# zhuker/lamejs

Hardware: NVIDIA H100
Metric: encoded audio seconds/sec (44.1kHz stereo 128kbps CBR) (higher is better)
Workload: dtype f64

## Files before the change

lamejs_b200/csrc/k_quant.cuh:

```cuda
#ifndef MP3B200_K_QUANT_CUH
#define MP3B200_K_QUANT_CUH
#include <stddef.h>
#include "mp3_device.cuh"
#include "mp3_tables.h"
#include "k_psy.cuh"

#define Q_LARGE_BITS 100000
#define Q_IXMAX 8206
#define Q_FULL 0xffffffffu

struct GranuleInfoDev {
  int global_gain, part2_3_length, part2_length, big_values, count1, scalefac_compress;
  int table_select[3], region0_count, region1_count, preflag, scalefac_scale, count1table_select, block_type;
  int subblock_gain[4];
  int count1bits, sfbmax, sfbdivide, sfb_lmax, psymax, psy_lmax, sfb_smin, max_nonzero_coeff;
  int scalefac[MP3_SFBMAX];
  int slen[4];
  int part_row;
  int pad_;
  double xrpow_max;
};
struct QuantFrameState {
  int stream, rel_frame;
  int in_old[2], in_step[2];
  int out_old[2], out_step[2];
  int bs_gain0[2], bs_step0[2];
  int used0[2];
  unsigned long long bs_hash[2][2];
  int scfsi[2][4];
  int redo;
  int valid;
};
#define Q_R0(ch) (1 << (ch))
#define Q_R1S(ch) (4 << (ch))
#define Q_R1(ch) (16 << (ch))
#define Q_R0_ANY 3
#define Q_R1_ANY 48
#define Q_R1S_ANY 12
struct GcPrep { float xmin[MP3_SFBMAX]; int have, mnz, block_type; double xrpow_max; };

__device__ unsigned short g_huff_code[1666];
__device__ unsigned char g_huff_len[1666];
__constant__ int c_huff_off[34];
__constant__ int c_huff_xlen[34];
__device__ int g_t32l[16];
__device__ int g_t33l[16];
__constant__ int c_slen1_n[16];
__constant__ int c_slen2_n[16];
__device__ int g_slen_n[2][16];
__device__ int g_scale_tab[2][16];
__device__ unsigned int g_cat_tab[8][256];
__constant__ int c_slen1_tab[16];
__constant__ int c_slen2_tab[16];
__constant__ int c_huf_noesc[15];

static int quant_upload_constants() {
  static const int t32l[16] = {1, 5, 5, 7, 5, 8, 7, 9, 5, 7, 7, 9, 7, 9, 9, 10};
  static const int t33l[16] = {4, 5, 5, 6, 5, 6, 6, 7, 5, 6, 6, 7, 6, 7, 7, 8};
  static const int s1n[16] = {1, 1, 1, 1, 8, 2, 2, 2, 4, 4, 4, 8, 8, 8, 16, 16};
  static const int s2n[16] = {1, 2, 4, 8, 1, 2, 4, 8, 2, 4, 8, 2, 4, 8, 4, 8};
  static const int s1t[16] = {0, 0, 0, 0, 3, 1, 1, 1, 2, 2, 2, 3, 3, 3, 4, 4};
  static const int s2t[16] = {0, 1, 2, 3, 0, 1, 2, 3, 1, 2, 3, 1, 2, 3, 2, 3};
  static const int ss[16] = {0, 18, 36, 54, 54, 36, 54, 72, 54, 72, 90, 72, 90, 108, 108, 126};
  static const int sl[16] = {0, 10, 20, 30, 33, 21, 31, 41, 32, 42, 52, 43, 53, 63, 64, 74};
  static const int hn[15] = {1, 2, 5, 7, 7, 10, 10, 13, 13, 13, 13, 13, 13, 13, 13};
#define UP(sym, src) if (cudaMemcpyToSymbol(sym, src, sizeof(src)) != cudaSuccess) return -100
  UP(g_huff_code, MP3_HUFF_CODE); UP(g_huff_len, MP3_HUFF_LEN); UP(c_huff_off, MP3_HUFF_OFF);
  UP(c_huff_xlen, MP3_HUFF_XLEN);
  UP(g_t32l, t32l); UP(g_t33l, t33l); UP(c_slen1_n, s1n); UP(c_slen2_n, s2n);
  UP(c_slen1_tab, s1t); UP(c_slen2_tab, s2t); UP(c_huf_noesc, hn);
  {
    static int sn[2][16], st[2][16];
    static unsigned int ct[8][256];
    for (int k = 0; k < 16; k++) { sn[0][k] = s1n[k]; sn[1][k] = s2n[k]; st[0][k] = sl[k]; st[1][k] = ss[k]; }
    static const int fam[6] = {1, 2, 5, 7, 10, 13};
    for (int x = 0; x < 16; x++) for (int y = 0; y < 16; y++) {
      const int q = x * 16 + y;
      for (int c = 0; c < 6; c++) {
        const int t1 = fam[c], xl = MP3_HUFF_XLEN[t1];
        unsigned a = 0, b = 0, d = 0;
        if (x < xl && y < xl) {
          const int i = x * xl + y;
          if (c == 0) a = b = d = MP3_HUFF_LEN[MP3_HUFF_OFF[1] + i];
          else if (c == 1) { a = MP3_HUFF_TABLE23[i] >> 16; b = d = MP3_HUFF_TABLE23[i] & 0xffff; }
          else if (c == 2) { a = MP3_HUFF_TABLE56[i] >> 16; b = d = MP3_HUFF_TABLE56[i] & 0xffff; }
          else { a = MP3_HUFF_LEN[MP3_HUFF_OFF[t1] + i]; b = MP3_HUFF_LEN[MP3_HUFF_OFF[t1 + 1] + i]; d = MP3_HUFF_LEN[MP3_HUFF_OFF[t1 + 2] + i]; }
        }
        ct[c][q] = a | (b << 11) | (d << 22);
      }
      { const unsigned a = MP3_HUFF_LARGETBL[q] >> 16, b = MP3_HUFF_LARGETBL[q] & 0xffff; ct[6][q] = a | (b << 11) | (b << 22); }
      ct[7][q] = 0;
    }
    UP(g_slen_n, sn); UP(g_scale_tab, st); UP(g_cat_tab, ct);
  }
#undef UP
  return 0;
}

struct __align__(16) GcWork {
  float xrpow[576];
  short ixw[576];
  short* ixg;
  GranuleInfoDev w, b;
  const Mp3Geo* geo;
  float xmin[MP3_SFBMAX], distort[MP3_SFBMAX];
  int pn_step[MP3_SFBMAX]; float pn_noise[MP3_SFBMAX], pn_noise_log[MP3_SFBMAX];
  int pn_global_gain, pn_sfb_count1;
  unsigned char mode[MP3_SFBMAX + 1];
  short nstart[MP3_SFBMAX], nlen[MP3_SFBMAX];
  int scratch[8];
  double dscratch[4];
  __align__(16) float xr[576];
};
struct __align__(16) WarpShared {
  double ath[6];
  int scfsi[4];
  GcWork wk;
};
#define Q_STRIDE_NOXR ((int)((offsetof(WarpShared, wk) + offsetof(GcWork, xr) + 15) & ~(size_t)15))
static_assert((offsetof(WarpShared, wk) + offsetof(GcWork, xr)) % 16 == 0 && (offsetof(WarpShared, wk) + offsetof(GcWork, xrpow)) % 16 == 0 &&
              (offsetof(WarpShared, wk) + offsetof(GcWork, ixw)) % 16 == 0 && sizeof(WarpShared) % 16 == 0, "rows are moved as 16-byte vectors");
#ifndef Q_SLIM_BLOCKS
#define Q_SLIM_BLOCKS 9
#endif

#define LANE (threadIdx.x & 31)
#ifdef Q_TASKSTAT
__device__ int g_taskstat[1 << 16][8];
#endif
#ifdef Q_STATS
__device__ unsigned long long g_qstats[16];
#define QSTAT(i) do { if (LANE == 0) atomicAdd(&g_qstats[i], 1ull); } while (0)
#else
#define QSTAT(i) do { } while (0)
#endif
#define Q_PRAGMA(x) _Pragma(#x)
#define Q_UNROLL(n) Q_PRAGMA(unroll n)
#ifndef Q_RT_UNROLL
#define Q_RT_UNROLL 1
#endif
#ifndef Q_CB_UNROLL
#define Q_CB_UNROLL 1
#endif
#ifndef Q_CN_UNROLL
#define Q_CN_UNROLL 2
#endif
#ifndef Q_HELPER
#define Q_HELPER __forceinline__
#endif
#ifndef Q_SPEC_START
#define Q_SPEC_START 180
#endif
#ifndef Q_SPEC_STEP
#define Q_SPEC_STEP 32
#endif
#ifndef Q_SPEC_GR1_STEP
#define Q_SPEC_GR1_STEP 2
#endif
#ifndef Q_SPEC_FOLD
#define Q_SPEC_FOLD 1
#endif
#ifndef Q_MIN_BLOCKS
#define Q_MIN_BLOCKS 14
#endif
__device__ __noinline__ double q_log10(double x) { return m3_log10(x); }
__device__ __noinline__ double q_pow(double x, double y) { return m3_pow(x, y); }
__device__ __forceinline__ int wmax(int v) { return __reduce_max_sync(Q_FULL, v); }
__device__ __forceinline__ int wsum(int v) { return __reduce_add_sync(Q_FULL, v); }
__device__ __forceinline__ unsigned wsumu(unsigned v) { return __reduce_add_sync(Q_FULL, v); }

struct RegionClass { int cat; unsigned lin; int t1, t2; };
__device__ Q_HELPER RegionClass region_class(int mx) {
  RegionClass rc;
  rc.lin = 0; rc.t2 = 0;
  if (mx == 0) { rc.cat = 7; rc.t1 = 0; }
  else if (mx <= 15) {
    rc.t1 = c_huf_noesc[mx - 1];
    rc.cat = mx <= 3 ? mx - 1 : (mx <= 5 ? 3 : (mx <= 7 ? 4 : 5));
  } else {
    const int n = 32 - __clz(mx - 15);
    rc.t2 = 24 + (int)((0x7777665432100000ull >> (4 * n)) & 15ull);
    rc.t1 = max(rc.t2 - 8, 16 + (int)((0x7777766554432100ull >> (4 * n)) & 15ull));
    const unsigned la = (unsigned)c_huff_xlen[rc.t1], lb = (unsigned)c_huff_xlen[rc.t2];
    rc.lin = la | (lb << 11) | (lb << 22);
    rc.cat = 6;
// ... 149 lines not shown
    for (int p = lane; p < 288; p += 32) {
      unsigned v = 0;
      if (2 * p < qend) {
        const float2 xp = *reinterpret_cast<const float2*>(&wk->xrpow[2 * p]);
        double x0 = (double)xp.x * istep, x1 = (double)xp.y * istep;
        x0 += (double)__ldg(&T->adj43[js_trunc<DOM_TRUNC_QUANT>(x0)]);
        x1 += (double)__ldg(&T->adj43[js_trunc<DOM_TRUNC_QUANT>(x1)]);
        v = (unsigned)js_trunc<DOM_TRUNC_QUANT>(x0) | ((unsigned)js_trunc<DOM_TRUNC_QUANT>(x1) << 16);
        DOMAIN_MISS(DOM_PACK_SEARCH, x0 >= 32768.0 || x1 >= 32768.0);
        if (v != 0 && p < i0h) top = 2 * p + 2;
      }
      iw32[p] = v;
    }
    __syncwarp();
    return noquant_count_bits_w(T, ix, gi, wk, false, top);
  }
  const bool prev_data_use = use_prev && (gi->global_gain == wk->pn_global_gain);
  const bool calc_step = prev_data_use || gi->block_type == BT_NORM;
  int term = sfbmax + 1;
#pragma unroll 1
  for (int s0 = 0; s0 <= sfbmax; s0 += 32) {
    const int sfb = s0 + lane;
    int md = 0, trunc_here = 0;
    if (sfb <= sfbmax) {
      const int jst = wk->geo->start[sfb];
      const int step = calc_step ? sfb_step(gi, wk, sfb) : -1;
      if (prev_data_use && wk->pn_step[sfb] == step) md = 0;
      else {
        if (jst + wk->geo->width[sfb] > mnz) trunc_here = 1;
        md = (use_prev && wk->pn_sfb_count1 > 0 && sfb >= wk->pn_sfb_count1 && wk->pn_step[sfb] > 0 && step >= wk->pn_step[sfb]) ? 2 : 1;
      }
      wk->mode[sfb] = (unsigned char)md;
      wk->nstart[sfb] = jst;
    }
    const unsigned m = __ballot_sync(Q_FULL, trunc_here);
    if (m && term == sfbmax + 1) term = s0 + __ffs(m) - 1;
  }
  __syncwarp();
  int zero_from = 576;
  if (term <= sfbmax) {
    const int term_len = mnz - wk->nstart[term] + 1;
    zero_from = term_len > 0 ? ((term_len & 1) ? mnz : mnz + 1) : mnz;
    if (lane == 0) wk->mode[term] = 1;
  }
  __syncwarp();
  const double compare01 = T->cmp01_over_istep[gi->global_gain];
  int top = 0;
Q_UNROLL(Q_CB_UNROLL)
  for (int p = lane; p < 288; p += 32) {
    const int i = 2 * p;
    unsigned v;
    if (i >= zero_from) { v = 0; iw32[p] = 0; }
    else {
      const int md = wk->mode[wk->geo->sfb_of_line[i]];
      const bool z1 = (i + 1) >= zero_from;
      if (md == 0) {
        v = iw32[p];
        if (z1) { v &= 0xffffu; iw32[p] = v; }
      } else {
        const float2 xp = *reinterpret_cast<const float2*>(&wk->xrpow[i]);
        unsigned v0, v1;
        if (md == 2) { v0 = (compare01 > (double)xp.x) ? 0u : 1u; v1 = (compare01 > (double)xp.y) ? 0u : 1u; }
        else {
          double x0 = (double)xp.x * istep, x1 = (double)xp.y * istep;
          x0 += (double)__ldg(&T->adj43[js_trunc<DOM_TRUNC_QUANT>(x0)]);
          x1 += (double)__ldg(&T->adj43[js_trunc<DOM_TRUNC_QUANT>(x1)]);
          v0 = (unsigned)js_trunc<DOM_TRUNC_QUANT>(x0); v1 = (unsigned)js_trunc<DOM_TRUNC_QUANT>(x1);
          DOMAIN_MISS(DOM_PACK_OUTER, x0 >= 32768.0 || x1 >= 32768.0);
        }
        if (z1) v1 = 0;
        v = v0 | (v1 << 16);
        iw32[p] = v;
      }
    }
    if (v != 0 && p < i0h) top = 2 * p + 2;
  }
  __syncwarp();
  return noquant_count_bits_w(T, ix, gi, wk, use_prev, top);
}

struct NoiseRes { int over_count; double over_SSD, max_noise; int bits; };
__device__ __forceinline__ void calc_noise_w(const Mp3Tables* T, GcWork* wk, const GranuleInfoDev* gi, const short* ix, NoiseRes* res) {
  const int lane = LANE;
  const int psymax = gi->psymax, mnz = gi->max_nonzero_coeff;
  int first_trunc = psymax;
#pragma unroll 1
  for (int s0 = 0; s0 < psymax; s0 += 32) {
    const int sfb = s0 + lane;
    int crosses = 0;
    if (sfb < psymax) {
      const int j = wk->geo->start[sfb], w = wk->geo->width[sfb];
      if (wk->pn_step[sfb] == sfb_step(gi, wk, sfb)) wk->nlen[sfb] = -1;
      else { wk->nstart[sfb] = (short)j; wk->nlen[sfb] = (short)(w >> 1); crosses = (j + w) > mnz; }
    }
    const unsigned m = __ballot_sync(Q_FULL, crosses);
    if (m && first_trunc == psymax) first_trunc = s0 + __ffs(m) - 1;
  }
  __syncwarp();
  if (lane == 0 && first_trunc < psymax) {
    int j = wk->geo->start[first_trunc];
#pragma unroll 1
    for (int sfb = first_trunc; sfb < psymax; sfb++) {
      const int w = wk->geo->width[sfb];
      if (wk->nlen[sfb] < 0) { j += w; continue; }
      int l = w >> 1;
      if ((j + w) > mnz) { const int us = mnz - j + 1; l = us > 0 ? us >> 1 : 0; }
      wk->nstart[sfb] = (short)j; wk->nlen[sfb] = (short)l;
      j += 2 * l;
    }
  }
  __syncwarp();
  int over = 0, ssd = 0; double mxn = -20.0;
#pragma unroll 1
  for (int s0 = 0; s0 < psymax; s0 += 32) {
    const int sfb = s0 + lane;
    if (sfb < psymax) {
      const int s = sfb_step(gi, wk, sfb);
      const bool cached = wk->nlen[sfb] < 0;
      double noise;
      if (cached) noise = (double)wk->pn_noise[sfb];
      else {
        const double step = (double)T->pow20[s + MP3_QMAX2];
        int j = wk->nstart[sfb];
        noise = 0;
Q_UNROLL(Q_CN_UNROLL)
        for (int l = wk->nlen[sfb]; l > 0; l--, j += 2) {
          const float2 x = *reinterpret_cast<const float2*>(&wk->xr[j]);
          const unsigned q0 = reinterpret_cast<const unsigned short*>(ix)[j], q1 = reinterpret_cast<const unsigned short*>(ix)[j + 1];
          double temp;
          temp = fabs((double)x.x) - (double)__ldg(&T->pow43[q0]) * step; noise += temp * temp;
          temp = fabs((double)x.y) - (double)__ldg(&T->pow43[q1]) * step; noise += temp * temp;
        }
        wk->pn_step[sfb] = s;
        { f32s t; t = noise; wk->pn_noise[sfb] = t.v; }
      }
      noise = noise / (double)wk->xmin[sfb];
      { f32s t; t = noise; wk->distort[sfb] = t.v; }
      if (cached) noise = (double)wk->pn_noise_log[sfb];
      else {
        noise = q_log10(js_dmax(noise, 1E-20));
        { f32s t; t = noise; wk->pn_noise_log[sfb] = t.v; }
      }
      if (noise > 0.0) {
        int tmp = js_trunc<DOM_TRUNC_NOISE>(noise * 10 + .5);
        if (tmp < 1) tmp = 1;
        ssd += tmp * tmp;
        over++;
      }
      mxn = js_dmax(mxn, noise);
    }
  }
#pragma unroll 1
  for (int o = 16; o > 0; o >>= 1) {
    const double other = __shfl_xor_sync(Q_FULL, mxn, o);
    mxn = js_dmax(mxn, other);
  }
  over = wsum(over);
  if (lane == 0) wk->pn_global_gain = gi->global_gain;
  __syncwarp();
  res->over_count = over; res->over_SSD = (double)wsum(ssd); res->max_noise = mxn;
}

__device__ __forceinline__ bool scale_bitcount_w(GranuleInfoDev* gi) {
  const int lane = LANE;
  int* scalefac = gi->scalefac;
  const bool is_short = gi->block_type == BT_SHORT;
  const int sfbmax = gi->sfbmax, sfbdivide = gi->sfbdivide;
  __syncwarp();
  if (!is_short && 0 == gi->preflag) {
    const bool in = lane >= 11 && lane < 21;
    const int pt = pretab_of(lane);
    const bool ok = !in || scalefac[lane] >= pt;
    if (__all_sync(Q_FULL, ok)) {
      __syncwarp();
      if (in) scalefac[lane] -= pt;
      if (lane == 0) gi->preflag = 1;
      __syncwarp();
    }
  }
  int m1 = 0, m2 = 0;
#pragma unroll 1
  for (int sfb = lane; sfb < sfbmax; sfb += 32) {
    const int v = scalefac[sfb];
    if (sfb < sfbdivide) m1 = max(m1, v); else m2 = max(m2, v);
  }
  m1 = wmax(m1); m2 = wmax(m2);
  int key = Q_LARGE_BITS * 16 + 15;
  if (lane < 16 && m1 < __ldg(&g_slen_n[0][lane]) && m2 < __ldg(&g_slen_n[1][lane])) key = __ldg(&g_scale_tab[is_short ? 1 : 0][lane]) * 16 + lane;
  key = __reduce_min_sync(Q_FULL, key);
  const int p2 = key >> 4;
  if (lane == 0) { gi->part2_length = p2; if (p2 != Q_LARGE_BITS) gi->scalefac_compress = key & 15; }
  __syncwarp();
  return p2 == Q_LARGE_BITS;
}

__device__ __forceinline__ bool scale_bitcount_lsf_w(GranuleInfoDev* gi) {
  const int lane = LANE;
  const bool is_short = gi->block_type == BT_SHORT;
  __syncwarp();
  int m0 = 0, m1 = 0, m2 = 0, m3 = 0;
  const int n = is_short ? 36 : 21;
#pragma unroll 1
  for (int i = lane; i < n; i += 32) {
    const int v = gi->scalefac[i];
    const int p = is_short ? i / 9 : (i < 6 ? 0 : (i - 6) / 5 + 1);
    if (p == 0) m0 = max(m0, v); else if (p == 1) m1 = max(m1, v); else if (p == 2) m2 = max(m2, v); else m3 = max(m3, v);
  }
  m0 = wmax(m0); m1 = wmax(m1); m2 = wmax(m2); m3 = wmax(m3);
  const bool over = m0 > 15 || m1 > 15 || m2 > 7 || m3 > 7;
  if (!over && lane == 0) {
// ... 916 lines not shown
      if (ixq[i + 2] != 0) { p += 2; huffbits *= 2; if (QNEG(i + 2)) huffbits++; }
      if (ixq[i + 3] != 0) { p++; huffbits *= 2; if (QNEG(i + 3)) huffbits++; }
      const int len = __ldg(&g_huff_len[c_huff_off[tb] + p]);
      if (pass == 0) mybits += len;
      else { put_bits(buf, at, (unsigned)huffbits + __ldg(&g_huff_code[c_huff_off[tb] + p]), len); at += len; }
    }
  }
  __syncwarp();
}

__device__ __forceinline__ void put_header_bits(unsigned int* buf, int pos, int val, int n) {
  while (n > 0) {
    const int k = min(n, 8 - (pos & 7));
    n -= k;
    const unsigned byte = ((unsigned)(val >> n) << (8 - (pos & 7) - k)) & 0xffu;
    const int b = pos >> 3;
    atomicOr(&buf[b >> 2], byte << (24 - 8 * (b & 3)));
    pos += k;
  }
}

__device__ __noinline__ void pack_sideinfo(const Mp3Tables* T, unsigned int* buf, const GranuleInfoDev* __restrict__ fin,
                                           const int* scfsi, int padding) {
  int p = 0;
#define WH(v, n) do { put_header_bits(buf, p, (int)(v), (n)); p += (n); } while (0)
  const int nch = T->nch;
  WH(T->mpeg25 ? 0xffe : 0xfff, 12); WH(T->version, 1); WH(4 - 3, 2); WH(1, 1);
  WH(T->bitrate_index, 4); WH(T->samplerate_index, 2); WH(padding, 1); WH(0, 1);
  WH(T->mono ? 3 : 0, 2); WH(0, 2); WH(0, 1); WH(1, 1); WH(0, 2);
  if (T->version == 1) {
    WH(0, 9);
    WH(0, nch == 2 ? 3 : 5);
#pragma unroll 1
    for (int ch = 0; ch < nch; ch++) for (int b = 0; b < 4; b++) WH(scfsi[ch * 4 + b], 1);
  } else {
    WH(0, 8);
    WH(0, nch);
  }
#pragma unroll 1
  for (int gr = 0; gr < T->mode_gr; gr++) for (int ch = 0; ch < nch; ch++) {
    const GranuleInfoDev* gi = &fin[gr * nch + ch];
    WH(gi->part2_3_length + gi->part2_length, 12);
    WH(gi->big_values / 2, 9);
    WH(gi->global_gain, 8);
    WH(gi->scalefac_compress, T->version == 1 ? 4 : 9);
    int ts0 = gi->table_select[0], ts1 = gi->table_select[1], ts2 = gi->table_select[2];
    if (ts0 == 14) ts0 = 16;
    if (ts1 == 14) ts1 = 16;
    if (gi->block_type != BT_NORM) {
      WH(1, 1); WH(gi->block_type, 2); WH(0, 1);
      WH(ts0, 5); WH(ts1, 5);
      WH(gi->subblock_gain[0], 3); WH(gi->subblock_gain[1], 3); WH(gi->subblock_gain[2], 3);
    } else {
      WH(0, 1);
      if (ts2 == 14) ts2 = 16;
      WH(ts0, 5); WH(ts1, 5); WH(ts2, 5);
      WH(gi->region0_count, 4); WH(gi->region1_count, 3);
    }
    if (T->version == 1) WH(gi->preflag, 1);
    WH(gi->scalefac_scale, 1); WH(gi->count1table_select, 1);
  }
#undef WH
}

__device__ __forceinline__ int granule_budget(int nch, int mean_bits, int gr, int used0, int used1, int ch) {
  int tbits = mean_bits;
  if (gr == 1) {
    const int resv = -(used0 + (nch == 2 ? used1 : 0)) + mean_bits;
    if (resv * 10 > 0) tbits += resv;
  }
  double t = (double)tbits / nch;
  if (t > 4095) t = 4095;
  int targ = (int)t;
  const int bits = targ * nch;
  if (bits > 7680) { targ = targ * 7680; targ = (int)((double)targ / bits); }
  (void)ch;
  return targ;
}

#ifndef Q_WARPS
#define Q_WARPS 4
#endif
#ifndef Q_BLOCKS_PER_SM
#define Q_BLOCKS_PER_SM 7
#endif
#define Q_THREADS (32 * Q_WARPS)

__device__ __forceinline__ int next_task(int* counter) {
  int t = 0;
  if (LANE == 0) t = atomicAdd(counter, 1);
  return __shfl_sync(Q_FULL, t, 0);
}
template <int STRIDE = (int)sizeof(WarpShared)>
__device__ __forceinline__ WarpShared* warp_shared() {
  extern __shared__ __align__(16) unsigned char smem_raw[];
  return reinterpret_cast<WarpShared*>(smem_raw + (threadIdx.x >> 5) * STRIDE);
}
__device__ __forceinline__ void gi_init_w(GranuleInfoDev* gi, const GcPrep* __restrict__ pr) {
  __syncwarp();
  int* w = reinterpret_cast<int*>(gi);
#pragma unroll 1
  for (int i = LANE; i < (int)(sizeof(GranuleInfoDev) / 4); i += 32) w[i] = 0;
  __syncwarp();
  if (LANE == 0) {
    const int bt = pr->block_type;
    const bool is_short = bt == BT_SHORT;
    gi->global_gain = 210; gi->block_type = bt;
    gi->sfb_lmax = is_short ? 0 : 21; gi->sfb_smin = is_short ? 0 : 12; gi->psy_lmax = is_short ? 0 : 21;
    gi->psymax = is_short ? 36 : 21; gi->sfbmax = is_short ? 36 : 21; gi->sfbdivide = is_short ? 18 : 11;
    gi->max_nonzero_coeff = pr->mnz; gi->xrpow_max = pr->xrpow_max;
  }
  __syncwarp();
}
__device__ __forceinline__ void copy_row16_w(void* dst, const void* src, int nbytes) {
  __syncwarp();
  const int n = nbytes >> 4;
  int4 v[5];
#pragma unroll
  for (int k = 0; k < 5; k++) { const int i = LANE + 32 * k; if (i < n) v[k] = reinterpret_cast<const int4*>(src)[i]; }
#pragma unroll
  for (int k = 0; k < 5; k++) { const int i = LANE + 32 * k; if (i < n) reinterpret_cast<int4*>(dst)[i] = v[k]; }
  __syncwarp();
}
struct FrameGeom { int z, f, padding, frame_bytes, mean_bits; long long kabs; };
__device__ __forceinline__ FrameGeom frame_geom(const Mp3Tables* T, const StreamDesc* streams, const QuantFrameState* q) {
  FrameGeom g;
  g.z = q->stream; g.f = q->rel_frame;
  g.kabs = (long long)streams[g.z].frame0 + g.f;
  g.padding = (int)(pad_count(g.kabs, T->frac_SpF, T->samplerate) - pad_count(g.kabs - 1, T->frac_SpF, T->samplerate));
  g.frame_bytes = T->frame_bytes_nopad + g.padding;
  g.mean_bits = (8 * g.frame_bytes - T->sideinfo_len * 8) / T->mode_gr;
  return g;
}

__global__ void __launch_bounds__(Q_THREADS, Q_BLOCKS_PER_SM)
k_q_prepare(const Mp3Tables* __restrict__ T, const StreamDesc* __restrict__ streams, const float* __restrict__ xr,
            const PsyRatioDev* __restrict__ ratio, const signed char* __restrict__ bt_final, const double* __restrict__ ath_q,
            const QuantFrameState* __restrict__ qs, float* __restrict__ xrq, float* __restrict__ xrpow_g, unsigned* __restrict__ neg_g,
            GcPrep* __restrict__ prep,
            int nframes, int* __restrict__ counter) {
  WarpShared* ws = warp_shared();
  GcWork* wk = &ws->wk;
  const int lane = LANE, nch = T->nch;
  const int G = T->mode_gr;
  const int ntasks = nframes * G * nch;
#pragma unroll 1
  for (int t = next_task(counter); t < ntasks; t = next_task(counter)) {
    const int frow = t / (G * nch), rem = t - frow * G * nch, gr = rem / nch, ch = rem - gr * nch;
    const QuantFrameState* q = qs + frow;
    const int z = q->stream, f = q->rel_frame;
    const StreamDesc& sd = streams[z];
    const double ath_adjust = ath_q[frow];
    const size_t urow = (size_t)sd.unit_base + G * f + gr, gidx = urow * nch + ch;
    const int bt = bt_final[urow * 2 + ch];
    const PsyRatioDev* rt = ratio + ((size_t)sd.unit_base + z + G * f + gr) * nch + ch;
    __syncwarp();
    if (lane < 6) ws->ath[lane] = ath_adjust_dev(ath_adjust, (double)(bt == BT_SHORT ? T->ath_psfb12[lane] : T->ath_psfb21[lane]), T->ath_floor);
    __syncwarp();
    const bool have = gc_prepare_w(T, wk, ws->ath, xr + gidx * 576, bt, rt, ath_adjust);
    copy_row16_w(xrq + gidx * 576, wk->xr, 2304);
    {
      unsigned mine = 0;
#pragma unroll 1
      for (int k = 0; k < 18; k++) { const unsigned m = __ballot_sync(Q_FULL, wk->xr[lane + 32 * k] < 0.0f); if (lane == k) mine = m; }
      if (lane < 18) neg_g[gidx * 18 + lane] = mine;
    }
    copy_row16_w(xrpow_g + gidx * 576, wk->xrpow, 2304);
    GcPrep* pr = prep + gidx;
#pragma unroll 1
    for (int i = lane; i < MP3_SFBMAX; i += 32) pr->xmin[i] = wk->xmin[i];
    if (lane == 0) { pr->have = have ? 1 : 0; pr->mnz = wk->b.max_nonzero_coeff; pr->block_type = bt; pr->xrpow_max = wk->b.xrpow_max; }
  }
}

__global__ void __launch_bounds__(Q_THREADS, Q_SLIM_BLOCKS)
k_q_search(const Mp3Tables* __restrict__ T, const StreamDesc* __restrict__ streams, QuantFrameState* __restrict__ qs,
           GranuleInfoDev* __restrict__ ginfo, short* __restrict__ l3enc, const float* __restrict__ xrpow_g,
           const GcPrep* __restrict__ prep, int gr, const int* __restrict__ list, const int* __restrict__ count_ptr, int count_direct,
           int revalidate, int* __restrict__ counter, int* __restrict__ list2, int* __restrict__ count2,
           int* __restrict__ list3, int* __restrict__ count3) {
  WarpShared* ws = warp_shared<Q_STRIDE_NOXR>();
  GcWork* wk = &ws->wk;
  const int lane = LANE, nch = T->nch;
  const int ntasks = (count_ptr ? *count_ptr : count_direct) * nch;
#pragma unroll 1
  for (int t = next_task(counter); t < ntasks; t = next_task(counter)) {
    const int wi = t / nch, ch = t - wi * nch;
    const int frow = list ? list[wi] : wi;
    QuantFrameState* q = qs + frow;
    const int flags = revalidate ? q->redo : 0;
    if (revalidate == 3 && (flags & Q_R0_ANY)) continue;
    if (revalidate && gr == 1 && !(flags & (Q_R0_ANY | Q_R1S(ch)))) continue;
    const FrameGeom fg = frame_geom(T, streams, q);
    const StreamDesc& sd = streams[fg.z];
    const size_t urow = (size_t)sd.unit_base + T->mode_gr * fg.f + gr, gidx = urow * nch + ch;
    const int targ = granule_budget(nch, fg.mean_bits, gr, q->used0[0], q->used0[1], ch);
    int ov = gr == 0 ? q->in_old[ch] : q->bs_gain0[ch];
    int cs = gr == 0 ? q->in_step[ch] : q->bs_step0[ch];
    const GcPrep* pr = prep + gidx;
    const bool have = pr->have != 0;
    gi_init_w(&wk->b, pr);
    if (lane == 0) wk->geo = &T->geo[pr->block_type == BT_SHORT ? 1 : 0];
    unsigned long long h = 0;
    if (have) {
      copy_row16_w(wk->xrpow, xrpow_g + gidx * 576, 2304);
      QSTAT(revalidate ? 12 + gr : 11);
      bin_search_w(T, wk, targ, &ov, &cs, revalidate ? 2 + 2 * gr : 0);
      h = gi_hash(&wk->b);
    } else {
      __syncwarp();
#pragma unroll 1
      for (int i = lane; i < 288; i += 32) reinterpret_cast<unsigned*>(wk->ixw)[i] = 0;
      __syncwarp();
    }
    bool store;
    if (!revalidate) {
      store = true;
      if (gr == 0 && fg.f != 0 && T->mode_gr == 2) cs = Q_SPEC_GR1_STEP;
      if (lane == 0) {
        q->bs_hash[gr][ch] = h;
        if (gr == 0) { q->bs_gain0[ch] = ov; q->bs_step0[ch] = cs; }
        if (gr == T->mode_gr - 1) { q->out_old[ch] = ov; q->out_step[ch] = cs; }
      }
    } else if (gr == 0) {
      store = ov != q->bs_gain0[ch] || h != q->bs_hash[0][ch];
      const bool step_changed = cs != q->bs_step0[ch];
      __syncwarp();
      if (lane == 0) {
        int old = -1;
        if (T->mode_gr == 1) { q->out_old[ch] = ov; q->out_step[ch] = cs; }
        if (store) {
          q->bs_gain0[ch] = ov; q->bs_step0[ch] = cs; q->bs_hash[0][ch] = h; old = atomicOr(&q->redo, Q_R0(ch));
          if ((old & Q_R0_ANY) == 0) list3[atomicAdd(count3, 1)] = frow;
        } else if (step_changed && T->mode_gr == 2) { q->bs_step0[ch] = cs; old = atomicOr(&q->redo, Q_R1S(ch)); }
        if (old == 0) list2[atomicAdd(count2, 1)] = frow;
      }
    } else {
      store = (flags & Q_R0_ANY) || ov != q->out_old[ch] || h != q->bs_hash[1][ch];
      __syncwarp();
      if (lane == 0) {
        q->out_step[ch] = cs;
        if (store) { q->out_old[ch] = ov; q->bs_hash[1][ch] = h; atomicOr(&q->redo, Q_R1(ch)); }
      }
    }
    if (store) {
      copy_row16_w(l3enc + gidx * 576, wk->ixw, 1152);
      copy_gi_w(&ginfo[gidx], &wk->b);
    }
  }
}

__global__ void __launch_bounds__(Q_THREADS, Q_BLOCKS_PER_SM)
k_q_outer(const Mp3Tables* __restrict__ T, const StreamDesc* __restrict__ streams, QuantFrameState* __restrict__ qs,
          GranuleInfoDev* __restrict__ ginfo, short* __restrict__ l3enc, const float* __restrict__ xrq,
          const float* __restrict__ xrpow_g, const GcPrep* __restrict__ prep, int gr, const int* __restrict__ list,
          const int* __restrict__ count_ptr, int count_direct, int revalidate, int* __restrict__ counter) {
  WarpShared* ws = warp_shared();
  GcWork* wk = &ws->wk;
  const int lane = LANE, nch = T->nch;
  const int ntasks = (count_ptr ? *count_ptr : count_direct) * nch;
#pragma unroll 1
  for (int t = next_task(counter); t < ntasks; t = next_task(counter)) {
    const int wi = t / nch, ch = t - wi * nch;
#ifdef Q_REVERSE
    const int frow = list ? list[wi] : (ntasks / nch - 1 - wi);
#else
    const int frow = list ? list[wi] : wi;
#endif
    QuantFrameState* q = qs + frow;
    if (revalidate == 1 && !(q->redo & (gr == 0 ? Q_R0(ch) : Q_R1(ch)))) continue;
    if (revalidate == -1 && (q->redo & Q_R0_ANY)) continue;
    if (revalidate > 0) QSTAT(14);
    const FrameGeom fg = frame_geom(T, streams, q);
    const StreamDesc& sd = streams[fg.z];
    const size_t urow = (size_t)sd.unit_base + T->mode_gr * fg.f + gr, gidx = urow * nch + ch;
    const int targ = granule_budget(nch, fg.mean_bits, gr, q->used0[0], q->used0[1], ch);
    const GcPrep* pr = prep + gidx;
    const bool have = pr->have != 0;
    short* const ixrow = l3enc + gidx * 576;
    __syncwarp();
    if (lane == 0) { wk->geo = &T->geo[pr->block_type == BT_SHORT ? 1 : 0]; wk->ixg = ixrow; }
    copy_gi_w(&wk->b, &ginfo[gidx]);
    copy_row16_w(wk->ixw, ixrow, 1152);
#ifdef Q_TASKSTAT
    const long long ts_t0 = clock64();
    const int ts_gain = wk->b.global_gain, ts_bits = wk->b.part2_3_length;
#endif
    if (have) {
      copy_row16_w(wk->xr, xrq + gidx * 576, 2304);
      copy_row16_w(wk->xrpow, xrpow_g + gidx * 576, 2304);
#pragma unroll 1
      for (int i = lane; i < MP3_SFBMAX; i += 32) wk->xmin[i] = pr->xmin[i];
      __syncwarp();
      outer_loop_w(T, wk, targ);
    }
#ifdef Q_TASKSTAT
    if (lane == 0 && revalidate <= 0 && gidx < (1u << 16)) {
      int* r = g_taskstat[gidx];
      r[0] = (int)((clock64() - ts_t0) >> 6); r[1] = gr; r[2] = wk->b.max_nonzero_coeff; r[3] = wk->b.block_type;
      r[4] = ts_gain; r[5] = ts_bits; r[6] = targ; r[7] = wk->b.global_gain;
    }
#endif
    copy_gi_w(&ginfo[gidx], &wk->b);
    copy_row16_w(ixrow, wk->ixw, 1152);
  }
}

__global__ void __launch_bounds__(Q_THREADS, Q_SLIM_BLOCKS)
k_q_finish(const Mp3Tables* __restrict__ T, const StreamDesc* __restrict__ streams, QuantFrameState* __restrict__ qs,
           GranuleInfoDev* __restrict__ ginfo, short* __restrict__ l3enc, int gr, const int* __restrict__ list,
           const int* __restrict__ count_ptr, int count_direct, int revalidate, int* __restrict__ counter) {
  WarpShared* ws = warp_shared<Q_STRIDE_NOXR>();
  GcWork* wk = &ws->wk;
  const int lane = LANE, nch = T->nch;
  const int ntasks = (count_ptr ? *count_ptr : count_direct) * nch;
#pragma unroll 1
  for (int t = next_task(counter); t < ntasks; t = next_task(counter)) {
    const int wi = t / nch, ch = t - wi * nch;
    const int frow = list ? list[wi] : wi;
    QuantFrameState* q = qs + frow;
    if (revalidate == 1 && !(q->redo & (gr == 0 ? Q_R0(ch) : Q_R1(ch)))) continue;
    if (revalidate == -1 && (q->redo & Q_R0_ANY)) continue;
    const StreamDesc& sd = streams[q->stream];
    const size_t urow = (size_t)sd.unit_base + T->mode_gr * q->rel_frame + gr, gidx = urow * nch + ch;
    short* const ixrow = l3enc + gidx * 576;
    copy_gi_w(&wk->b, &ginfo[gidx]);
    copy_row16_w(wk->ixw, ixrow, 1152);
    if (lane == 0) wk->geo = &T->geo[wk->b.block_type == BT_SHORT ? 1 : 0];
    __syncwarp();
    best_scalefac_store_w(wk, ws->scfsi, gr == 1 ? &ginfo[gidx - nch] : nullptr, gr, T->mode_gr);
    best_huffman_divide_w(T, wk);
    copy_gi_w(&ginfo[gidx], &wk->b);
    if (gr == 0) { if (lane == 0) q->used0[ch] = wk->b.part2_3_length + wk->b.part2_length; }
    else if (lane < 4) q->scfsi[ch][lane] = ws->scfsi[lane];
  }
}

struct __align__(16) PackShared {
  unsigned int bits[368];
  short ix[576];
  unsigned neg[20];
  GranuleInfoDev gi;
  int scfsi[8];
};
__global__ void __launch_bounds__(Q_THREADS)
k_q_pack(const Mp3Tables* __restrict__ T, const StreamDesc* __restrict__ streams, QuantFrameState* __restrict__ qs,
         const GranuleInfoDev* __restrict__ ginfo, const short* __restrict__ l3enc, const unsigned* __restrict__ neg_g,
         const int* __restrict__ list, const int* __restrict__ count_ptr, int count_direct, int revalidate,
         int* __restrict__ counter, uint8_t* __restrict__ out, int* __restrict__ over_budget) {
  extern __shared__ __align__(16) unsigned char smem_raw[];
  PackShared* ps = reinterpret_cast<PackShared*>(smem_raw) + (threadIdx.x >> 5);
  const int lane = LANE, nch = T->nch;
  const int ntasks = count_ptr ? *count_ptr : count_direct;
#pragma unroll 1
  for (int t = next_task(counter); t < ntasks; t = next_task(counter)) {
    const int frow = list ? list[t] : t;
    QuantFrameState* q = qs + frow;
    if (revalidate && !(q->redo & (Q_R0_ANY | Q_R1_ANY))) continue;
    if (revalidate) QSTAT(5);
    const FrameGeom fg = frame_geom(T, streams, q);
    const StreamDesc& sd = streams[fg.z];
    const size_t g0 = ((size_t)sd.unit_base + T->mode_gr * fg.f) * nch;
    int used = 0;
#pragma unroll 1
    for (int k = 0; k < T->mode_gr * nch; k++) used += ginfo[g0 + k].part2_3_length + ginfo[g0 + k].part2_length;
    const bool over = used > 8 * (fg.frame_bytes - T->sideinfo_len);
    if (lane == 0 && over != (q->valid == 2)) atomicAdd(over_budget, over ? 1 : -1);
    if (over) { if (lane == 0) q->valid = 2; continue; }
    __syncwarp();
#pragma unroll 1
    for (int i = lane; i < 368; i += 32) ps->bits[i] = 0;
    if (lane < 8) ps->scfsi[lane] = q->scfsi[lane >> 2][lane & 3];
    __syncwarp();
    int pos = 8 * T->sideinfo_len;
#pragma unroll 1
    for (int k = 0; k < T->mode_gr * nch; k++) {
      copy_gi_w(&ps->gi, &ginfo[g0 + k]);
      copy_row16_w(ps->ix, l3enc + (g0 + k) * 576, 1152);
      if (lane < 18) ps->neg[lane] = neg_g[(g0 + k) * 18 + lane];
      __syncwarp();
      pack_gc_w(T, ps->bits, &ps->gi, ps->ix, ps->neg, pos);
      pos += ps->gi.part2_3_length + ps->gi.part2_length;
      __syncwarp();
    }
    if (lane == 0) {
      pack_sideinfo(T, ps->bits, ginfo + g0, ps->scfsi, fg.padding);
      int remaining = 8 * fg.frame_bytes - pos;
// ... 26 lines not shown
    q->out_old[c] = q->out_step[c] = 0;
    q->used0[c] = 0; q->bs_gain0[c] = q->bs_step0[c] = 0;
    for (int b = 0; b < 4; b++) q->scfsi[c][b] = 0;
  }
}

__global__ void k_qstate_verify(const StreamDesc* __restrict__ streams, QuantFrameState* __restrict__ qs, long long nframes,
                                int* __restrict__ list, int* __restrict__ counter, int predict_step) {
  const long long r = (long long)blockIdx.x * blockDim.x + threadIdx.x;
  if (r >= nframes) return;
  QuantFrameState* q = qs + r;
  if (q->rel_frame == 0) return;
  const QuantFrameState* p = q - 1;
  int pstep[2] = {p->out_step[0], p->out_step[1]};
  if (predict_step && p->rel_frame != 0) {
    const QuantFrameState* pp = p - 1;
#pragma unroll 1
    for (int c = 0; c < 2; c++) pstep[c] = (pp->out_old[c] - p->out_old[c] >= 4) ? 4 : 2;
  }
  bool same = true;
#pragma unroll 1
  for (int c = 0; c < 2; c++) if (q->in_old[c] != p->out_old[c] || q->in_step[c] != pstep[c]) same = false;
  if (!same) {
#pragma unroll 1
    for (int c = 0; c < 2; c++) { q->in_old[c] = p->out_old[c]; q->in_step[c] = pstep[c]; }
    q->redo = 0;
    list[atomicAdd(counter, 1)] = (int)r;
  }
}

__global__ void k_qstate_commit(StreamDesc* __restrict__ streams, int nstreams, const QuantFrameState* __restrict__ qs) {
  const int z = blockIdx.x * blockDim.x + threadIdx.x;
  if (z >= nstreams) return;
  StreamDesc& sd = streams[z];
  if (sd.nframes <= 0) return;
  const QuantFrameState* q = qs + sd.frame_base + sd.nframes - 1;
#pragma unroll 1
  for (int c = 0; c < 2; c++) { sd.old_value[c] = q->out_old[c]; sd.current_step[c] = q->out_step[c]; }
}

__global__ void k_qstate_loop_cond(cudaGraphConditionalHandle loop, int* __restrict__ count, int* __restrict__ st, int max_passes) {
  const int n = *count;
  int passes = st[2];
  bool more = n != 0;
  if (more) passes++;
  if (passes > max_passes) { st[1] = 1; *count = 0; more = false; }
  st[2] = passes;
  if (passes > st[0]) st[0] = passes;
  cudaGraphSetConditional(loop, more ? 1u : 0u);
}

struct QuantBuffers {
  const float* xr; const PsyRatioDev* ratio; const signed char* bt; const double* ath_q;
  QuantFrameState* qs; GranuleInfoDev* ginfo; short* l3enc; float* xrq; float* xrpow; unsigned* neg; GcPrep* prep;
  int* over_budget;
  int* list; int* counter;
};
#define Q_NCOUNTERS 256
#define Q_REPAIR_BLOCKS 16
enum { QE_START, QE_PREP, QE_S0, QE_O0, QE_F0, QE_S1, QE_MID, QE_O1, QE_F1, QE_PK, QE_COUNT };

struct QuantLoop {
  cudaStream_t capture = nullptr;
  int* st = nullptr;
  cudaGraphExec_t exec = nullptr;
};

static int quant_run(const Mp3Tables* dT, const Mp3Tables& hT, StreamDesc* d_streams, int S, int nstreams_with_frames, int max_frames, long long F,
                     const QuantBuffers& B, uint8_t* d_out, cudaStream_t st_main, cudaStream_t st_repair, cudaEvent_t ev_fork, cudaEvent_t ev_join,
                     cudaEvent_t ev_pass1, cudaEvent_t* evq, int* evq_pred, int* passes_out, std::atomic<long long>* launches,
                     QuantLoop* dloop = nullptr) {
  cudaStream_t st = st_main;
  static std::mutex attr_mu;
  static bool attr_done[64] = {};
  int dev = 0, sms = 132;
  cudaGetDevice(&dev);
  cudaDeviceGetAttribute(&sms, cudaDevAttrMultiProcessorCount, dev);
  const size_t smem = sizeof(WarpShared) * Q_WARPS, smem_slim = (size_t)Q_STRIDE_NOXR * Q_WARPS, smem_pack = sizeof(PackShared) * Q_WARPS;
  {
    std::lock_guard<std::mutex> lk(attr_mu);
    if (dev < 64 && !attr_done[dev]) {
      if (cudaFuncSetAttribute(k_q_prepare, cudaFuncAttributeMaxDynamicSharedMemorySize, (int)smem) != cudaSuccess) return -100;
      if (cudaFuncSetAttribute(k_q_search, cudaFuncAttributeMaxDynamicSharedMemorySize, (int)smem_slim) != cudaSuccess) return -100;
      if (cudaFuncSetAttribute(k_q_outer, cudaFuncAttributeMaxDynamicSharedMemorySize, (int)smem) != cudaSuccess) return -100;
      if (cudaFuncSetAttribute(k_q_finish, cudaFuncAttributeMaxDynamicSharedMemorySize, (int)smem_slim) != cudaSuccess) return -100;
      if (cudaFuncSetAttribute(k_q_pack, cudaFuncAttributeMaxDynamicSharedMemorySize, (int)smem_pack) != cudaSuccess) return -100;
      attr_done[dev] = true;
    }
  }
  if (F <= 0) { *passes_out = 0; return 0; }
  const int nch = hT.nch;
  int next_counter = Q_NCOUNTERS;
  auto fresh_counter = [&]() -> int* {
    if (next_counter >= Q_NCOUNTERS) { cudaMemsetAsync(B.counter + 3, 0, sizeof(int) * (Q_NCOUNTERS - 3), st); next_counter = 3; }
    return B.counter + next_counter++;
  };
  auto grid_for = [&](long long tasks, int per_sm) -> int {
    long long g = (tasks + Q_WARPS - 1) / Q_WARPS, cap = (long long)sms * per_sm;
    if (g > cap) g = cap;
    return (int)(g < 1 ? 1 : g);
  };
  {
    dim3 g((max_frames + 127) / 128, S);
    k_qstate_init<<<g, 128, 0, st>>>(d_streams, S, B.qs);
    (*launches)++;
  }
  for (int i = 0; i < QE_COUNT; i++) evq_pred[i] = -1;
  int last_slot = -1;
  auto mark = [&](int slot) { cudaEventRecord(evq[slot], st); evq_pred[slot] = last_slot; last_slot = slot; };
  int* const prep_counter = fresh_counter();
  mark(QE_START);
  k_q_prepare<<<grid_for(F * hT.mode_gr * nch, Q_BLOCKS_PER_SM), Q_THREADS, smem, st>>>(dT, d_streams, B.xr, B.ratio, B.bt, B.ath_q, B.qs, B.xrq, B.xrpow, B.neg,
                                                                              B.prep, (int)F, prep_counter);
  mark(QE_PREP);
  (*launches)++;
  int* const list1 = B.list;
  int* const list2 = B.list + (F + 1);
  int* const list3 = B.list + 2 * (F + 1);
  auto search = [&](int gr, const int* list, const int* cptr, long long count, int reval) {
    k_q_search<<<grid_for(count * nch, Q_SLIM_BLOCKS), Q_THREADS, smem_slim, st>>>(dT, d_streams, B.qs, B.ginfo, B.l3enc, B.xrpow, B.prep, gr, list, cptr, (int)count,
                                                                             reval, fresh_counter(), list2, B.counter + 1, list3, B.counter + 2);
    (*launches)++;
  };
  int reserve_blocks = 0;
  auto finish = [&](int gr, const int* list, const int* cptr, long long count, int reval) {
    k_q_finish<<<max(1, grid_for(count * nch, Q_SLIM_BLOCKS) - reserve_blocks), Q_THREADS, smem_slim, st>>>(dT, d_streams, B.qs, B.ginfo, B.l3enc, gr, list, cptr, (int)count, reval, fresh_counter());
    (*launches)++;
  };
  auto outer = [&](int gr, const int* list, const int* cptr, long long count, int reval) {
    k_q_outer<<<max(1, grid_for(count * nch, Q_BLOCKS_PER_SM) - reserve_blocks), Q_THREADS, smem, st>>>(dT, d_streams, B.qs, B.ginfo, B.l3enc, B.xrq, B.xrpow, B.prep, gr, list, cptr, (int)count,
                                                                            reval, fresh_counter());
    (*launches)++;
  };
  auto outer_finish = [&](int gr, long long count, int reval, int slot_o, int slot_f) {
    outer(gr, nullptr, nullptr, count, reval); mark(slot_o);
    finish(gr, nullptr, nullptr, count, reval); mark(slot_f);
  };
  auto pack = [&](const int* list, const int* cptr, long long count, int reval) {
    k_q_pack<<<grid_for(count, 9), Q_THREADS, smem_pack, st>>>(dT, d_streams, B.qs, B.ginfo, B.l3enc, B.neg, list, cptr, (int)count, reval, fresh_counter(), d_out, B.over_budget);
    (*launches)++;
  };
  auto verify = [&](int predict_step = 0) {
    cudaMemsetAsync(B.counter, 0, 3 * sizeof(int), st);
    k_qstate_verify<<<(int)((F + 255) / 256), 256, 0, st>>>(d_streams, B.qs, F, list1, B.counter, predict_step);
    (*launches)++;
  };
  const int G = hT.mode_gr;
  const bool speculated = F > nstreams_with_frames;
  search(0, nullptr, nullptr, F, 0); mark(QE_S0);
  if (G == 2) {
    outer_finish(0, F, 0, QE_O0, QE_F0);
    search(1, nullptr, nullptr, F, 0); mark(QE_S1);
  }
  bool forked = false;
  if (Q_SPEC_FOLD && speculated) {
    verify(G == 1 ? 1 : 0);
    search(0, list1, B.counter, F, 1);
    if (G == 2) {
      search(1, list2, B.counter + 1, F, 3);
      int* const c0 = fresh_counter(); int* const c1 = fresh_counter(); int* const c2 = fresh_counter();
      int* const c3 = fresh_counter(); int* const c4 = fresh_counter();
      cudaEventRecord(ev_fork, st_main);
      cudaStreamWaitEvent(st_repair, ev_fork, 0);
      const int gq = Q_REPAIR_BLOCKS, gs = Q_REPAIR_BLOCKS;
      const int* cp = B.counter + 2;
      k_q_outer<<<gq, Q_THREADS, smem, st_repair>>>(dT, d_streams, B.qs, B.ginfo, B.l3enc, B.xrq, B.xrpow, B.prep, 0, list3, cp, (int)F, 1, c0);
      k_q_finish<<<gs, Q_THREADS, smem_slim, st_repair>>>(dT, d_streams, B.qs, B.ginfo, B.l3enc, 0, list3, cp, (int)F, 1, c1);
      k_q_search<<<gs, Q_THREADS, smem_slim, st_repair>>>(dT, d_streams, B.qs, B.ginfo, B.l3enc, B.xrpow, B.prep, 1, list3, cp, (int)F, 1, c2, list2, B.counter + 1,
                                                          list3, B.counter + 2);
      k_q_outer<<<gq, Q_THREADS, smem, st_repair>>>(dT, d_streams, B.qs, B.ginfo, B.l3enc, B.xrq, B.xrpow, B.prep, 1, list3, cp, (int)F, 2, c3);
      k_q_finish<<<gs, Q_THREADS, smem_slim, st_repair>>>(dT, d_streams, B.qs, B.ginfo, B.l3enc, 1, list3, cp, (int)F, 2, c4);
      cudaEventRecord(ev_join, st_repair);
      (*launches) += 5;
      forked = true;
    }
  }
  mark(QE_MID);
  if (G == 2) {
    reserve_blocks = forked ? Q_REPAIR_BLOCKS : 0;
    outer_finish(1, F, forked ? -1 : 0, QE_O1, QE_F1);
    reserve_blocks = 0;
    if (forked) cudaStreamWaitEvent(st_main, ev_join, 0);
  } else {
    outer_finish(0, F, 0, QE_O0, QE_F0);
  }
  pack(nullptr, nullptr, F, 0); mark(QE_PK);
  if (cudaEventRecord(ev_pass1, st) != cudaSuccess) return -100;
  int passes = 2;
  auto revalidate = [&](const int* count1, long long count) {
    search(0, list1, count1, count, 1);
    outer(0, list2, B.counter + 1, count, 1);
    finish(0, list2, B.counter + 1, count, 1);
    if (G == 2) {
      search(1, list2, B.counter + 1, count, 1);
      outer(1, list2, B.counter + 1, count, 1);
      finish(1, list2, B.counter + 1, count, 1);
    }
    pack(list2, B.counter + 1, count, 1);
  };
  if (dloop && speculated) {
    if (!dloop->exec) {
      cudaGraph_t g = nullptr;
      cudaGraphConditionalHandle cond;
      cudaGraphNode_t reset, loop;
      cudaMemsetParams mp = {};
      mp.dst = dloop->st + 2; mp.value = 2; mp.elementSize = sizeof(int); mp.width = 1; mp.height = 1;
      cudaGraphNodeParams cp = {};
      cp.type = cudaGraphNodeTypeConditional;
      if (cudaGraphCreate(&g, 0) != cudaSuccess) return -100;
      bool ok = cudaGraphConditionalHandleCreate(&cond, g, 1, cudaGraphCondAssignDefault) == cudaSuccess &&
                cudaGraphAddMemsetNode(&reset, g, nullptr, 0, &mp) == cudaSuccess;
      cp.conditional.handle = cond; cp.conditional.type = cudaGraphCondTypeWhile; cp.conditional.size = 1;
      ok = ok && cudaGraphAddNode(&loop, g, &reset, 1, &cp) == cudaSuccess;
      cudaGraph_t body = ok ? cp.conditional.phGraph_out[0] : nullptr;
      if (ok && cudaStreamBeginCaptureToGraph(dloop->capture, body, nullptr, nullptr, 0, cudaStreamCaptureModeThreadLocal) == cudaSuccess) {
        std::atomic<long long> captured{0};
        std::atomic<long long>* const counted = launches;
        launches = &captured;
        st = dloop->capture;
        next_counter = Q_NCOUNTERS;
        verify();
        k_qstate_loop_cond<<<1, 1, 0, st>>>(cond, B.counter, dloop->st, max_frames + 3);
        revalidate(B.counter, F);
        st = st_main;
        launches = counted;
        cudaGraph_t captured_body = nullptr;
        ok = cudaStreamEndCapture(dloop->capture, &captured_body) == cudaSuccess && captured_body == body &&
             cudaGraphInstantiate(&dloop->exec, g, 0) == cudaSuccess;
      } else {
        ok = false;
      }
      cudaGraphDestroy(g);
      if (!ok) { dloop->exec = nullptr; return -100; }
    }
    if (cudaGraphLaunch(dloop->exec, st) != cudaSuccess) return -100;
    (*launches)++;
  }
  for (; speculated && !dloop;) {
    verify();
    int h_count = 0;
    if (cudaMemcpyAsync(&h_count, B.counter, sizeof(int), cudaMemcpyDeviceToHost, st) != cudaSuccess) return -100;
    if (cudaStreamSynchronize(st) != cudaSuccess) return -100;
    if (h_count == 0) break;
    revalidate(nullptr, h_count);
    passes++;
    if (passes > max_frames + 3) return -100;
  }
  k_qstate_commit<<<(S + 63) / 64, 64, 0, st>>>(d_streams, S, B.qs);
  (*launches)++;
  *passes_out = passes;
  return 0;
}

// ... 2 lines not shown
```

Before: 57690.

## Read xr from global in outer loop, shrink outer smem, raise occupancy

The outer-loop kernel no longer copies the 2304-byte xr row into shared memory; calc_noise reads it from global through the read-only cache via a per-warp pointer. This lets k_q_outer launch with the slim shared-memory stride, and its launch bounds and grid sizing now target 9 blocks per SM, while prepare keeps 7 through a new separate constant. The noise loop now pays L1/L2 latency instead of shared-memory latency, traded for higher occupancy and one less row copy per task. The task count is also moved into shared memory, and a zero-init of the copy register is added.

```diff
diff --git a/lamejs_b200/csrc/k_quant.cuh b/lamejs_b200/csrc/k_quant.cuh
--- a/lamejs_b200/csrc/k_quant.cuh
+++ b/lamejs_b200/csrc/k_quant.cuh
@@ -101,6 +101,9 @@
   float xrpow[576];
   short ixw[576];
   short* ixg;
+  GranuleInfoDev* gig;
+  const float* xrg;
+  int ntasks;
   GranuleInfoDev w, b;
   const Mp3Geo* geo;
   float xmin[MP3_SFBMAX], distort[MP3_SFBMAX];
@@ -416,6 +419,7 @@
 struct NoiseRes { int over_count; double over_SSD, max_noise; int bits; };
 __device__ __forceinline__ void calc_noise_w(const Mp3Tables* T, GcWork* wk, const GranuleInfoDev* gi, const short* ix, NoiseRes* res) {
   const int lane = LANE;
+  const float* __restrict__ xr = wk->xrg;
   const int psymax = gi->psymax, mnz = gi->max_nonzero_coeff;
   int first_trunc = psymax;
 #pragma unroll 1
@@ -459,7 +463,7 @@
         noise = 0;
 Q_UNROLL(Q_CN_UNROLL)
         for (int l = wk->nlen[sfb]; l > 0; l--, j += 2) {
-          const float2 x = *reinterpret_cast<const float2*>(&wk->xr[j]);
+          const float2 x = __ldg(reinterpret_cast<const float2*>(xr + j));
           const unsigned q0 = reinterpret_cast<const unsigned short*>(ix)[j], q1 = reinterpret_cast<const unsigned short*>(ix)[j + 1];
           double temp;
           temp = fabs((double)x.x) - (double)__ldg(&T->pow43[q0]) * step; noise += temp * temp;
@@ -1542,7 +1546,10 @@
 #define Q_WARPS 4
 #endif
 #ifndef Q_BLOCKS_PER_SM
-#define Q_BLOCKS_PER_SM 7
+#define Q_BLOCKS_PER_SM 9
+#endif
+#ifndef Q_PREP_BLOCKS
+#define Q_PREP_BLOCKS 7
 #endif
 #define Q_THREADS (32 * Q_WARPS)
 
@@ -1576,6 +1583,7 @@
   __syncwarp();
   const int n = nbytes >> 4;
   int4 v[5];
+  v[4] = make_int4(0, 0, 0, 0);
 #pragma unroll
   for (int k = 0; k < 5; k++) { const int i = LANE + 32 * k; if (i < n) v[k] = reinterpret_cast<const int4*>(src)[i]; }
 #pragma unroll
@@ -1593,7 +1601,7 @@
   return g;
 }
 
-__global__ void __launch_bounds__(Q_THREADS, Q_BLOCKS_PER_SM)
+__global__ void __launch_bounds__(Q_THREADS, Q_PREP_BLOCKS)
 k_q_prepare(const Mp3Tables* __restrict__ T, const StreamDesc* __restrict__ streams, const float* __restrict__ xr,
             const PsyRatioDev* __restrict__ ratio, const signed char* __restrict__ bt_final, const double* __restrict__ ath_q,
             const QuantFrameState* __restrict__ qs, float* __restrict__ xrq, float* __restrict__ xrpow_g, unsigned* __restrict__ neg_g,
@@ -1715,15 +1723,16 @@
           GranuleInfoDev* __restrict__ ginfo, short* __restrict__ l3enc, const float* __restrict__ xrq,
           const float* __restrict__ xrpow_g, const GcPrep* __restrict__ prep, int gr, const int* __restrict__ list,
           const int* __restrict__ count_ptr, int count_direct, int revalidate, int* __restrict__ counter) {
-  WarpShared* ws = warp_shared();
+  WarpShared* ws = warp_shared<Q_STRIDE_NOXR>();
   GcWork* wk = &ws->wk;
   const int lane = LANE, nch = T->nch;
-  const int ntasks = (count_ptr ? *count_ptr : count_direct) * nch;
-#pragma unroll 1
-  for (int t = next_task(counter); t < ntasks; t = next_task(counter)) {
+  if (lane == 0) wk->ntasks = (count_ptr ? *count_ptr : count_direct) * nch;
+  __syncwarp();
+#pragma unroll 1
+  for (int t = next_task(counter); t < wk->ntasks; t = next_task(counter)) {
     const int wi = t / nch, ch = t - wi * nch;
 #ifdef Q_REVERSE
-    const int frow = list ? list[wi] : (ntasks / nch - 1 - wi);
+    const int frow = list ? list[wi] : (wk->ntasks / nch - 1 - wi);
 #else
     const int frow = list ? list[wi] : wi;
 #endif
@@ -1739,7 +1748,7 @@
     const bool have = pr->have != 0;
     short* const ixrow = l3enc + gidx * 576;
     __syncwarp();
-    if (lane == 0) { wk->geo = &T->geo[pr->block_type == BT_SHORT ? 1 : 0]; wk->ixg = ixrow; }
+    if (lane == 0) { wk->geo = &T->geo[pr->block_type == BT_SHORT ? 1 : 0]; wk->ixg = ixrow; wk->gig = &ginfo[gidx]; wk->xrg = xrq + gidx * 576; }
     copy_gi_w(&wk->b, &ginfo[gidx]);
     copy_row16_w(wk->ixw, ixrow, 1152);
 #ifdef Q_TASKSTAT
@@ -1747,7 +1756,6 @@
     const int ts_gain = wk->b.global_gain, ts_bits = wk->b.part2_3_length;
 #endif
     if (have) {
-      copy_row16_w(wk->xr, xrq + gidx * 576, 2304);
       copy_row16_w(wk->xrpow, xrpow_g + gidx * 576, 2304);
 #pragma unroll 1
       for (int i = lane; i < MP3_SFBMAX; i += 32) wk->xmin[i] = pr->xmin[i];
@@ -1761,8 +1769,8 @@
       r[4] = ts_gain; r[5] = ts_bits; r[6] = targ; r[7] = wk->b.global_gain;
     }
 #endif
-    copy_gi_w(&ginfo[gidx], &wk->b);
-    copy_row16_w(ixrow, wk->ixw, 1152);
+    copy_gi_w(wk->gig, &wk->b);
+    copy_row16_w(wk->ixg, wk->ixw, 1152);
   }
 }
 
@@ -1955,7 +1963,7 @@
     if (dev < 64 && !attr_done[dev]) {
       if (cudaFuncSetAttribute(k_q_prepare, cudaFuncAttributeMaxDynamicSharedMemorySize, (int)smem) != cudaSuccess) return -100;
       if (cudaFuncSetAttribute(k_q_search, cudaFuncAttributeMaxDynamicSharedMemorySize, (int)smem_slim) != cudaSuccess) return -100;
-      if (cudaFuncSetAttribute(k_q_outer, cudaFuncAttributeMaxDynamicSharedMemorySize, (int)smem) != cudaSuccess) return -100;
+      if (cudaFuncSetAttribute(k_q_outer, cudaFuncAttributeMaxDynamicSharedMemorySize, (int)smem_slim) != cudaSuccess) return -100;
       if (cudaFuncSetAttribute(k_q_finish, cudaFuncAttributeMaxDynamicSharedMemorySize, (int)smem_slim) != cudaSuccess) return -100;
       if (cudaFuncSetAttribute(k_q_pack, cudaFuncAttributeMaxDynamicSharedMemorySize, (int)smem_pack) != cudaSuccess) return -100;
       attr_done[dev] = true;
@@ -1983,7 +1991,7 @@
   auto mark = [&](int slot) { cudaEventRecord(evq[slot], st); evq_pred[slot] = last_slot; last_slot = slot; };
   int* const prep_counter = fresh_counter();
   mark(QE_START);
-  k_q_prepare<<<grid_for(F * hT.mode_gr * nch, Q_BLOCKS_PER_SM), Q_THREADS, smem, st>>>(dT, d_streams, B.xr, B.ratio, B.bt, B.ath_q, B.qs, B.xrq, B.xrpow, B.neg,
+  k_q_prepare<<<grid_for(F * hT.mode_gr * nch, Q_PREP_BLOCKS), Q_THREADS, smem, st>>>(dT, d_streams, B.xr, B.ratio, B.bt, B.ath_q, B.qs, B.xrq, B.xrpow, B.neg,
                                                                               B.prep, (int)F, prep_counter);
   mark(QE_PREP);
   (*launches)++;
@@ -2001,7 +2009,7 @@
     (*launches)++;
   };
   auto outer = [&](int gr, const int* list, const int* cptr, long long count, int reval) {
-    k_q_outer<<<max(1, grid_for(count * nch, Q_BLOCKS_PER_SM) - reserve_blocks), Q_THREADS, smem, st>>>(dT, d_streams, B.qs, B.ginfo, B.l3enc, B.xrq, B.xrpow, B.prep, gr, list, cptr, (int)count,
+    k_q_outer<<<max(1, grid_for(count * nch, Q_BLOCKS_PER_SM) - reserve_blocks), Q_THREADS, smem_slim, st>>>(dT, d_streams, B.qs, B.ginfo, B.l3enc, B.xrq, B.xrpow, B.prep, gr, list, cptr, (int)count,
                                                                             reval, fresh_counter());
     (*launches)++;
   };
@@ -2037,11 +2045,11 @@
       cudaStreamWaitEvent(st_repair, ev_fork, 0);
       const int gq = Q_REPAIR_BLOCKS, gs = Q_REPAIR_BLOCKS;
       const int* cp = B.counter + 2;
-      k_q_outer<<<gq, Q_THREADS, smem, st_repair>>>(dT, d_streams, B.qs, B.ginfo, B.l3enc, B.xrq, B.xrpow, B.prep, 0, list3, cp, (int)F, 1, c0);
+      k_q_outer<<<gq, Q_THREADS, smem_slim, st_repair>>>(dT, d_streams, B.qs, B.ginfo, B.l3enc, B.xrq, B.xrpow, B.prep, 0, list3, cp, (int)F, 1, c0);
       k_q_finish<<<gs, Q_THREADS, smem_slim, st_repair>>>(dT, d_streams, B.qs, B.ginfo, B.l3enc, 0, list3, cp, (int)F, 1, c1);
       k_q_search<<<gs, Q_THREADS, smem_slim, st_repair>>>(dT, d_streams, B.qs, B.ginfo, B.l3enc, B.xrpow, B.prep, 1, list3, cp, (int)F, 1, c2, list2, B.counter + 1,
                                                           list3, B.counter + 2);
-      k_q_outer<<<gq, Q_THREADS, smem, st_repair>>>(dT, d_streams, B.qs, B.ginfo, B.l3enc, B.xrq, B.xrpow, B.prep, 1, list3, cp, (int)F, 2, c3);
+      k_q_outer<<<gq, Q_THREADS, smem_slim, st_repair>>>(dT, d_streams, B.qs, B.ginfo, B.l3enc, B.xrq, B.xrpow, B.prep, 1, list3, cp, (int)F, 2, c3);
       k_q_finish<<<gs, Q_THREADS, smem_slim, st_repair>>>(dT, d_streams, B.qs, B.ginfo, B.l3enc, 1, list3, cp, (int)F, 2, c4);
       cudaEventRecord(ev_join, st_repair);
       (*launches) += 5;
```

New measurement: 59060, median of 6. No clear change (+2.4%).
